# dogeplusplus/torch-actor-critic

Measured on AMD Instinct MI355X. Metric: sac_updates_per_sec, higher is better.
Workload: dtype bf16; 1 GPU; model=SAC-MLP[256, 256]-HalfCheetah-v4, global_batch=64, seq_len=1, parallelism=dp1, obs_dim=17, act_dim=6, replay_buffer=1000000, update_window=50, graph=True, engine=fused, mode=full

## Files before the change

torch_actor_critic_amd/algo/engine.py:

```python

import logging
import math
import os
import typing as t

import torch

from ..buffer.replay import ReplayBuffer
from ..models.mlp import Actor, DoubleCritic
from ..optim import FlatAdam
from ..parallel import comm


_log = logging.getLogger(__name__)


class FusedSACEngine:
    def __init__(self, sac, actor: Actor, critic: DoubleCritic,
                 target_critic: DoubleCritic, buffer: ReplayBuffer,
                 pi_opt: FlatAdam, q_opt: FlatAdam,
                 target_flat: torch.Tensor, batch_size: int,
                 device: torch.device, sample: bool = True,
                 capture: bool = True, philox_seed: int = 0):
        from ..ops import require_extension
# ... 134 lines not shown
                             == "1" and not self._use_side)
        self._wjobs: t.List[tuple] = []
        adam_flag = os.environ.get("TAC_AMD_WGRAD_ADAM", "auto")
        self._wgrad_adam_unsplit = adam_flag == "1"
        self._wgrad_adam = (
            adam_flag != "0"
            and self.world == 1 and not self._force_coll
            and os.environ.get("TAC_AMD_SPLIT_GRAPHS") != "1"
            and self._wgrad_batch)
        self._adam_fused: t.Dict[int, bool] = {}
        self._wt_of = {
            w.grad.data_ptr(): wt
            for w, wt in zip(self._c_tr_src + self._a_tr_src,
                             self._c_tr_dst + self._a_tr_dst)}
        self._bump_fold = os.environ.get("TAC_AMD_BUMP_FOLD", "1") != "0"
        self._r1_dgrad = (
            os.environ.get("TAC_AMD_R1_DGRAD", "1") != "0"
            and len(self.c_w) >= 2 and not self._loss_fuse)
        if self._r1_dgrad and any(self.cwt[z][-1].data_ptr() % 16
                                  for z in range(2)):
            _log.info("engine: rank-1 dgrad operand off (last-layer W^T "
                      "row is not 16-byte aligned); keeping the K=1 launch")
            self._r1_dgrad = False
        self._s2 = torch.cuda.Stream()
        self._fork_evs = [torch.cuda.Event() for _ in range(12)]
        self._join_evs = [torch.cuda.Event() for _ in range(4)]
        self._ev_i = 0
        self._join_i = 0

        torch.cuda.synchronize()

        self._graphs = None
        self.graph = None
        if capture:
            self._capture()


    def _side(self, fn):
        if not self._use_side:
            fn()
            return
        ev = self._fork_evs[self._ev_i % len(self._fork_evs)]
        self._ev_i += 1
        ev.record()
        with torch.cuda.stream(self._s2):
            self._s2.wait_event(ev)
# ... 41 lines not shown
                        [j[6] for j in self._wjobs],
                        [j[7] for j in self._wjobs]) <= 1:
                why = ("the launch does not split along M "
                       "(TAC_AMD_WGRAD_ADAM=1 folds it anyway)")
            if why:
                _log.info("engine: Adam stays in adam_t for the %d-element "
                          "optimizer: %s", g.numel(), why)
            self._adam_fused[key] = why is None
        return self._adam_fused[key]

    def _wflush(self, opt=None, targ=None, rho=0.0):
        if not self._wjobs:
            return
        cols = [list(c) for c in zip(*self._wjobs)]
        if opt is not None and self._adam_covers(opt):
            wts = [self._wt_of.get(dw.data_ptr()) for dw in cols[3]]
            self.ext.mwgrad_het_adam(
                *cols, opt.fp.flat, opt.fp.flat_grad, opt.m, opt.v,
                opt.step_t, opt.lr, opt.betas[0], opt.betas[1], opt.eps,
                opt.weight_decay, wts, targ, rho)
        else:
            self.ext.mwgrad_het(*cols)
        self._wjobs = []

    def _mg(self, xs, ws, bs, ys, masks, M, N, K, lda, ldy, relu,
            xs2=None, ws2=None, masks2=None, K2=0, x_off=0, x2_off=0,
            x_offs=None):
        self.ext.mgemm(xs, ws, bs, ys, masks, M, N, K, lda, ldy, relu,
                       xs2 or [], ws2 or [], masks2 or [], K2, x_off,
                       x2_off, x_offs or [])

    def _critic_fwd(self, x_src, x_off, weights, acts, lda,
                    need_hidden_acts=True):
        B = self.B
        nL = len(self.c_w)
        if self.use_mlpf:
            e = self._empty
            act_arg = [
                [acts[z][i] if (need_hidden_acts or i == nL - 1) else e
                 for i in range(nL)] for z in range(2)]
            self.ext.mlp_fwd_fused(
                x_src, x_off, lda, B, self.OC,
                [[weights[z][i][0] for i in range(nL)] for z in range(2)],
                [[e] * nL for _ in range(2)],
                [[weights[z][i][1] for i in range(nL)] for z in range(2)],
                [[e] * nL for _ in range(2)],
# ... 95 lines not shown
                          self.c_act[0][i], self.c_act[1][i]],
                         [None] * 4, B, self.c_w[i], k, lda, self.c_w[i],
                         relu, x_offs=offs4)
                xs4 = [self.t_act[0][i], self.t_act[1][i],
                       self.c_act[0][i], self.c_act[1][i]]
                offs4 = [0, 0, 0, 0]
                k = self.c_w[i]
                lda = k
        else:
            self._critic_fwd(self.XC, B * self.OCp, self.tw, self.t_act,
                             self.OCp,
                             need_hidden_acts=False)
            self._critic_fwd(self.XC, 0, self.cw, self.c_act, self.OCp)

        nL = len(self.c_w)
        q = [self.c_act[z][nL - 1] for z in range(2)]
        qt = [self.t_act[z][nL - 1] for z in range(2)]
        fuse = self._loss_fuse
        bump = ((self.ctr, self.q_opt.step_t, self.pi_opt.step_t)
                if self._bump_fold else (None, None, None))
        buf = self.buffer
        per = ((self.pprob, buf._size_dev, buf._beta_dev, self.td)
               if self.per else ())
        ext.qloss2(q[0], q[1], qt[0], qt[1], self.logp[B:], self.rew,
                   self.done, self.alpha_dev, self.alpha_host,
                   self.loss_q_acc, self.dq[0], self.dq[1], B,
                   self.sac.gamma, self.sac.reward_scale,
                   self.cwt[0][nL - 1] if fuse else None,
                   self.cwt[1][nL - 1] if fuse else None,
                   self.dc[0][nL - 2] if fuse else None,
                   self.dc[1][nL - 2] if fuse else None,
                   self.c_w[nL - 2] if fuse else 0, *bump, *per)
        if self.per:
            ext.per_update(buf._per_tree, buf.max_size, self.idx, self.td,
                           buf.per_alpha, buf.per_eps, buf._max_priority)

        d = self.dq
        for i in range(nL - 1, -1, -1):
            relu_mask = i + 1 < nL
            masks = [self.c_act[z][i] if relu_mask else None
                     for z in range(2)]
            if i > 0:
                x_in = [self.c_act[z][i - 1] for z in range(2)]
                ldx, xoff = self.c_w[i - 1], 0
            else:
                x_in = [self.XC, self.XC]
                ldx, xoff = self.OCp, 0
            self._wgrad(list(d), list(masks), list(x_in),
                        [self.cw[z][i][0].grad for z in range(2)],
                        [self.cw[z][i][1].grad for z in range(2)],
                        B, self.c_w[i],
                        (self.c_w[i - 1] if i > 0 else OC),
                        self.c_w[i], ldx, xoff)
            if i > 0:
                if i == nL - 1 and fuse:
                    pass
                else:
                    self._mg(d, [self.cwt[z][i] for z in range(2)],
                             [None, None],
                             [self.dc[z][i - 1] for z in range(2)],
                             masks, B, self.c_w[i - 1], self.c_w[i],
                             self.c_w[i], self.c_w[i - 1], False)
                d = [self.dc[z][i - 1] for z in range(2)]
        self._wflush(self.q_opt, self.target_flat, self.sac.polyak)
        self._join_side()

    def _phase_policy(self):
        ext = self.ext
        B, O, A, OC = self.B, self.O, self.A, self.OC
        qo = self.q_opt
        if not self._adam_fused.get(id(qo), False):
            ext.adam_t(qo.fp.flat, qo.fp.flat_grad, qo.m, qo.v, qo.step_t,
                       qo.lr, qo.betas[0], qo.betas[1], qo.eps,
                       qo.weight_decay, self._c_offs, self._c_tr_dst,
                       self.target_flat, self.sac.polyak)

        self._critic_fwd(self.XC2, 0, self.cw, self.p_act, self.OCp)
        nL = len(self.c_w)
        qp = [self.p_act[z][nL - 1] for z in range(2)]
        fuse = self._loss_fuse
        ext.piloss2(qp[0], qp[1], self.logp[:B], self.alpha_dev,
                    self.alpha_host, self.loss_pi_acc, self.mean_logp,
                    self.dqp[0], self.dqp[1], B,
                    self.cwt[0][nL - 1] if fuse else None,
                    self.cwt[1][nL - 1] if fuse else None,
                    self.dcp[0][nL - 2] if fuse else None,
                    self.dcp[1][nL - 2] if fuse else None,
                    self.c_w[nL - 2] if fuse else 0)

        d = self.dqp
        r1 = None
        for i in range(nL - 1, 0, -1):
            masks = [self.p_act[z][i] if i + 1 < nL else None
                     for z in range(2)]
            if i == nL - 1 and fuse:
                d = [self.dcp[z][i - 1] for z in range(2)]
                continue
            if i == nL - 1 and self._r1_dgrad:
                r1 = (list(self.dqp),
                      [self.cwt[z][nL - 1] for z in range(2)])
                continue
            if r1 is not None:
                ext.mgemm_r1(r1[0], r1[1],
                             [self.cwt[z][i] for z in range(2)],
                             [self.dcp[z][i - 1] for z in range(2)], masks,
                             B, self.c_w[i - 1], self.c_w[i],
                             self.c_w[i - 1])
                r1 = None
            else:
                self._mg(d, [self.cwt[z][i] for z in range(2)],
                         [None, None],
                         [self.dcp[z][i - 1] for z in range(2)], masks,
                         B, self.c_w[i - 1], self.c_w[i], self.c_w[i],
                         self.c_w[i - 1], False)
            d = [self.dcp[z][i - 1] for z in range(2)]
        masks0 = [self.p_act[z][0] for z in range(2)]
        if r1 is not None:
            ext.mgemm_r1(r1[0], r1[1], [self.cwt[z][0] for z in range(2)],
                         [self.dxc, self.dxc2], masks0, B, OC, self.c_w[0],
                         self.OCp)
        else:
            self._mg(d, [self.cwt[z][0] for z in range(2)], [None, None],
                     [self.dxc, self.dxc2], masks0,
                     B, OC, self.c_w[0], self.c_w[0], self.OCp, False)

        ext.tg_bwd2(self.dxc, O, self.dxc2, self.alpha_dev,
                    self.alpha_host, self.hl, self.prob, self.dmu,
                    self.dls, B, self.act_limit, self.lo, self.hi)
        h_last = self.a_hidden[-1]
        a_last = self.a_act[-1]
        (wm, bm), (wl, bl) = self.head_w
        self._wgrad([self.dmu, self.dls], [None, None], [a_last, a_last],
                    [wm.grad, wl.grad], [bm.grad, bl.grad],
                    B, A, h_last, A, h_last, 0)
        self._mg([self.dmu], [self.hwt[0]], [None], [self.da[-1]], [None],
                 B, h_last, A, A, h_last, False,
                 xs2=[self.dls], ws2=[self.hwt[1]], masks2=[None], K2=A)

        d = self.da[-1]
        for i in range(len(self.aw) - 1, -1, -1):
            mask = self.a_act[i]
            if i > 0:
                x_in, ldx, xoff = self.a_act[i - 1], self.a_hidden[i - 1], 0
# ... 137 lines not shown
```

torch_actor_critic_amd/ops/csrc/fused.hip:

```cpp

#include <hip/hip_runtime.h>
#include <hip/hip_bf16.h>

#include <torch/extension.h>
#include <c10/hip/HIPStream.h>

#include <algorithm>
#include <utility>
#include <vector>

#include "replay_draw.h"

namespace fused {

using namespace replay;

using f32x4 = __attribute__((ext_vector_type(4))) float;
using bf16x8 = __attribute__((ext_vector_type(8))) __bf16;

__global__ __launch_bounds__(256)
void philox_words2_kernel(int64_t* __restrict__ out, uint64_t seed,
                          uint64_t chi, uint64_t clo0, int64_t n) {
  philox_words_row(out, seed, chi, clo0, n);
}
// ... 451 lines not shown
}

__global__ __launch_bounds__(256)
void mgemm_combine_kernel(MGemm g, int split, bool relu) {
  const int64_t per = (int64_t)g.M * g.N;
  const int64_t total = per * g.nz;
  const int64_t stride = (int64_t)gridDim.x * blockDim.x;
  for (int64_t i = (int64_t)blockIdx.x * blockDim.x + threadIdx.x;
       i < total; i += stride) {
    const int z = (int)(i / per);
    const int64_t off = i % per;
    float s = 0.f;
    for (int sl = 0; sl < split; ++sl)
      s += g.part[((int64_t)sl * g.nz + z) * per + off];
    const MProb& p = g.p[z];
    const int m = (int)(off / g.N), n = (int)(off % g.N);
    if (p.bias) s += p.bias[n];
    if (relu) s = fmaxf(s, 0.f);
    p.y[(int64_t)m * g.ldy + n] = s;
  }
}


constexpr int SKMAX = 256;
constexpr int SLPAD = 8;

DEVINL bool small_vec_ok(const float* src, const float* mask, int r0, int R,
                         int bound, int K, int ld) {
  return (r0 + R <= bound) && ((ld & 3) == 0) && ((K & 3) == 0)
         && ((((uintptr_t)src | (uintptr_t)mask) & 15) == 0);
}

template <int R, bool MASK, bool R1>
DEVINL void small_load(float (&v)[R], float (&mk)[MASK ? R : 1],
                       float (&ra)[R / 16], bool vec,
                       const float* src, const float* mask,
                       int r0, int bound, int K, int ld,
                       const float* r1c, const float* r1r) {
  const int tid = threadIdx.x;
  if (vec) {
    constexpr int G = 64 / R;
    constexpr int NQ = SKMAX / 16 / G;
    const int gr = r0 + ((tid >> 2) & (R - 1));
    const int kg = (tid >> 2) / R;
    const int c = tid & 3;
    if constexpr (R1) ra[0] = r1c[gr];
    const float* base = R1 ? r1r : src + (int64_t)gr * ld;
    const float* mbase = MASK ? mask + (int64_t)gr * ld : nullptr;
#pragma unroll
    for (int q = 0; q < NQ; ++q) {
      if (q * G * 16 < K) {
        const int col = min(((q * G + kg) * 4 + c) * 4, K - 4);
        float4 f = *(const float4*)(base + col);
        v[q*4+0] = f.x; v[q*4+1] = f.y; v[q*4+2] = f.z; v[q*4+3] = f.w;
        if constexpr (MASK) {
          float4 h = *(const float4*)(mbase + col);
          mk[q*4+0] = h.x; mk[q*4+1] = h.y; mk[q*4+2] = h.z; mk[q*4+3] = h.w;
        }
      } else {
#pragma unroll
        for (int j = 0; j < 4; ++j) {
          v[q*4+j] = 0.f;
          if constexpr (MASK) mk[q*4+j] = 0.f;
        }
      }
    }
  } else {
    const int rr = tid >> 4;
    const int cc = tid & 15;
#pragma unroll
    for (int p = 0; p < R / 16; ++p) {
      const bool rows_in = r0 + 16 * p < bound;
      const int gr = min(r0 + rr + 16 * p, bound - 1);
      if constexpr (R1) ra[p] = r1c[gr];
#pragma unroll
      for (int q = 0; q < SKMAX / 16; ++q) {
        if (rows_in && q * 16 < K) {
          const int col = min(cc + 16 * q, K - 1);
          if constexpr (R1) v[p*16+q] = r1r[col];
          else v[p*16+q] = src[(int64_t)gr * ld + col];
          if constexpr (MASK) mk[p*16+q] = mask[(int64_t)gr * ld + col];
        } else {
          v[p*16+q] = 0.f;
          if constexpr (MASK) mk[p*16+q] = 0.f;
        }
      }
    }
  }
}

template <int R, bool MASK, bool R1>
DEVINL void small_write(__bf16* d, int S, const float (&v)[R],
                        const float (&mk)[MASK ? R : 1],
                        const float (&ra)[R / 16], bool vec,
                        int r0, int bound, int K, int Kp) {
  const int tid = threadIdx.x;
  if (vec) {
// ... 19 lines not shown
      }
    }
  } else {
    const int rr = tid >> 4;
    const int cc = tid & 15;
#pragma unroll
    for (int p = 0; p < R / 16; ++p) {
      const int row = rr + 16 * p;
      const bool row_in = r0 + row < bound;
#pragma unroll
      for (int q = 0; q < SKMAX / 16; ++q) {
        if (q * 16 < Kp) {
          const int col = cc + 16 * q;
          float x = v[p*16+q];
          if constexpr (R1) x = ra[p] * x;
          if constexpr (MASK) x = mk[p*16+q] > 0.f ? x : 0.f;
          d[row * S + col] = (__bf16)((row_in && col < K) ? x : 0.f);
        }
      }
    }
  }
}

template <int TM, int TN, bool MASK, bool RELU, bool SUM2, bool R1>
__global__ __launch_bounds__(256)
void mgemm_small_kernel(MGemm g) {
  static_assert((TM == 32 || TM == 64) && (TN == 32 || TN == 64), "tile");
  static_assert(!(SUM2 && R1), "R1 has no second operand");
  constexpr int WM = TM / 2, WN = TN / 2;
  constexpr int MI = WM / 16, NI = WN / 16;
  constexpr int KT = SUM2 ? 2 * SKMAX : SKMAX;
  __shared__ __attribute__((aligned(16))) __bf16 smem[(TM + TN)
                                                      * (KT + SLPAD)];
  const MProb& p = g.p[blockIdx.z];
  const int tid = threadIdx.x;
  const int lane = tid & 63;
  const int wid = tid >> 6;
  const int wrow = (wid >> 1) * WM;
  const int wcol = (wid & 1) * WN;
  const int bm0 = blockIdx.x * TM;
  const int bn0 = blockIdx.y * TN;
  const int crow = (lane >> 4) * 4, ccol = lane & 15;

  const int Kp1 = (g.K + 31) & ~31;
  const int Kp2 = SUM2 ? ((g.K2 + 31) & ~31) : 0;
  const int S = Kp1 + Kp2 + SLPAD;
  __bf16* xs = smem;
  __bf16* ws = smem + TM * S;

  float bv[NI];
#pragma unroll
  for (int ni = 0; ni < NI; ++ni) {
    const int gcol = bn0 + wcol + ni * 16 + ccol;
    bv[ni] = (p.bias && gcol < g.N) ? p.bias[gcol] : 0.f;
  }
  float va[TM], ma[MASK ? TM : 1], ra[TM / 16], vb[TN], nomask[1],
        rb[TN / 16];
  const float* a_src = R1 ? p.r1_row : p.x;
  const bool veca = small_vec_ok(a_src, MASK ? p.mask : nullptr, bm0, TM,
                                 g.M, g.K, g.lda);
  const bool vecb = small_vec_ok(p.w, nullptr, bn0, TN, g.N, g.K, g.K);
  small_load<TM, MASK, R1>(va, ma, ra, veca, p.x, p.mask, bm0, g.M, g.K,
                           g.lda, p.r1_col, p.r1_row);
  small_load<TN, false, false>(vb, nomask, rb, vecb, p.w, nullptr, bn0, g.N,
                               g.K, g.K, nullptr, nullptr);
  float va2[SUM2 ? TM : 1], ma2[(SUM2 && MASK) ? TM : 1], vb2[SUM2 ? TN : 1];
  bool veca2 = false, vecb2 = false;
  if constexpr (SUM2) {
    veca2 = small_vec_ok(p.x2, MASK ? p.mask2 : nullptr, bm0, TM, g.M, g.K2,
                         g.K2);
    vecb2 = small_vec_ok(p.w2, nullptr, bn0, TN, g.N, g.K2, g.K2);
    small_load<TM, MASK, false>(va2, ma2, ra, veca2, p.x2, p.mask2, bm0, g.M,
                                g.K2, g.K2, nullptr, nullptr);
    small_load<TN, false, false>(vb2, nomask, rb, vecb2, p.w2, nullptr, bn0,
                                 g.N, g.K2, g.K2, nullptr, nullptr);
  }

  small_write<TM, MASK, R1>(xs, S, va, ma, ra, veca, bm0, g.M, g.K, Kp1);
  small_write<TN, false, false>(ws, S, vb, nomask, rb, vecb, bn0, g.N, g.K,
                                Kp1);
  if constexpr (SUM2) {
    small_write<TM, MASK, false>(xs + Kp1, S, va2, ma2, ra, veca2, bm0, g.M,
                                 g.K2, Kp2);
    small_write<TN, false, false>(ws + Kp1, S, vb2, nomask, rb, vecb2, bn0,
                                  g.N, g.K2, Kp2);
  }
  __syncthreads();

  f32x4 acc[MI][NI] = {};
  const int arow = lane & 15;
  const int ak0 = (lane >> 4) * 8;
  const __bf16* xr = xs + (wrow + arow) * S + ak0;
  const __bf16* wr = ws + (wcol + arow) * S + ak0;
  const int Kt = Kp1 + Kp2;
  for (int kk = 0; kk < Kt; kk += 32) {
    bf16x8 b[NI];
#pragma unroll
    for (int ni = 0; ni < NI; ++ni)
      b[ni] = *(const bf16x8*)&wr[ni * 16 * S + kk];
#pragma unroll
// ... 825 lines not shown

constexpr int LOSS_MAXB = 1024;

template <bool WEIGHTED>
__global__ __launch_bounds__(256)
void qloss2_kernel(const float* __restrict__ q1, const float* __restrict__ q2,
                   const float* __restrict__ q1t, const float* __restrict__ q2t,
                   const float* __restrict__ logp_next,
                   const float* __restrict__ rew, const float* __restrict__ done,
                   const float* __restrict__ alpha_dev, float alpha_host,
                   float* __restrict__ loss_acc,
                   float* __restrict__ dq1, float* __restrict__ dq2,
                   int B, float gamma, float scale,
                   const float* __restrict__ wt3_0,
                   const float* __restrict__ wt3_1,
                   float* __restrict__ dy2_0, float* __restrict__ dy2_1,
                   int h2,
                   int64_t* __restrict__ bump0, int64_t* __restrict__ bump1,
                   int64_t* __restrict__ bump2,
                   const float* __restrict__ prob,
                   const int64_t* __restrict__ size_dev,
                   const float* __restrict__ beta_dev,
                   float* __restrict__ td) {
  __shared__ float red[4];
  __shared__ float dqs[2][LOSS_MAXB];
  const float alpha = alpha_dev ? alpha_dev[0] : alpha_host;
  const bool fuse = dy2_0 != nullptr;
  int64_t c0 = 0, c1 = 0, c2 = 0;
  if (threadIdx.x == 0) {
    if (bump0) c0 = bump0[0];
    if (bump1) c1 = bump1[0];
    if (bump2) c2 = bump2[0];
  }
  float wsize = 0.f, nbeta = 0.f, wmax = 1.f;
  if constexpr (WEIGHTED) {
    __shared__ float redw[4];
    wsize = (float)size_dev[0];
    nbeta = -beta_dev[0];
    float m = 0.f;
    for (int i = threadIdx.x; i < B; i += blockDim.x)
      m = fmaxf(m, powf(wsize * prob[i], nbeta));
#pragma unroll
    for (int off = 32; off > 0; off >>= 1) m = fmaxf(m, __shfl_down(m, off));
    if ((threadIdx.x & 63) == 0) redw[threadIdx.x >> 6] = m;
    __syncthreads();
    wmax = fmaxf(fmaxf(redw[0], redw[1]), fmaxf(redw[2], redw[3]));
  }
  float acc = 0.f;
  for (int i = threadIdx.x; i < B; i += blockDim.x) {
    float backup = scale * rew[i] + gamma * (1.f - done[i]) *
                       (fminf(q1t[i], q2t[i]) - alpha * logp_next[i]);
    float e1 = q1[i] - backup, e2 = q2[i] - backup;
    float g1, g2;
    if constexpr (WEIGHTED) {
      const float w = powf(wsize * prob[i], nbeta) / wmax;
      acc += w * (e1 * e1 + e2 * e2);
      g1 = 2.f * (w * e1) / B;
      g2 = 2.f * (w * e2) / B;
      td[i] = 0.5f * (fabsf(e1) + fabsf(e2));
    } else {
      acc += e1 * e1 + e2 * e2;
      g1 = 2.f * e1 / B;
      g2 = 2.f * e2 / B;
    }
    dq1[i] = g1;
    dq2[i] = g2;
    if (fuse) { dqs[0][i] = g1; dqs[1][i] = g2; }
  }
#pragma unroll
  for (int off = 32; off > 0; off >>= 1) acc += __shfl_down(acc, off);
  if ((threadIdx.x & 63) == 0) red[threadIdx.x >> 6] = acc;
  __syncthreads();
  if (threadIdx.x == 0) {
    loss_acc[0] += (red[0] + red[1] + red[2] + red[3]) / B;
    if (bump0) bump0[0] = c0 + 1;
    if (bump1) bump1[0] = c1 + 1;
    if (bump2) bump2[0] = c2 + 1;
  }
  if (fuse) {
    const int64_t total = (int64_t)B * h2;
    for (int64_t idx = threadIdx.x; idx < total; idx += blockDim.x) {
      int i = (int)(idx / h2), j = (int)(idx % h2);
      dy2_0[idx] = dqs[0][i] * wt3_0[j];
      dy2_1[idx] = dqs[1][i] * wt3_1[j];
    }
  }
}

__global__ __launch_bounds__(256)
void piloss2_kernel(const float* __restrict__ q1, const float* __restrict__ q2,
                    const float* __restrict__ logp,
                    const float* __restrict__ alpha_dev, float alpha_host,
                    float* __restrict__ loss_acc,
                    float* __restrict__ mean_logp,
                    float* __restrict__ dq1, float* __restrict__ dq2,
                    int B,
                    const float* __restrict__ wt3_0,
                    const float* __restrict__ wt3_1,
                    float* __restrict__ dy2_0, float* __restrict__ dy2_1,
                    int h2) {
  __shared__ float red[4], redl[4];
  __shared__ float dqs[2][LOSS_MAXB];
  const float alpha = alpha_dev ? alpha_dev[0] : alpha_host;
  const bool fuse = dy2_0 != nullptr;
  float acc = 0.f, laux = 0.f;
  for (int i = threadIdx.x; i < B; i += blockDim.x) {
    float a = q1[i], b = q2[i];
    acc += alpha * logp[i] - fminf(a, b);
    laux += logp[i];
    float g1, g2;
    if (a < b)      { g1 = -1.f; g2 = 0.f; }
    else if (b < a) { g1 = 0.f;  g2 = -1.f; }
    else            { g1 = -0.5f; g2 = -0.5f; }
    dq1[i] = g1 / B;
    dq2[i] = g2 / B;
    if (fuse) { dqs[0][i] = g1 / B; dqs[1][i] = g2 / B; }
  }
#pragma unroll
  for (int off = 32; off > 0; off >>= 1) {
    acc += __shfl_down(acc, off);
    laux += __shfl_down(laux, off);
  }
  if ((threadIdx.x & 63) == 0) {
    red[threadIdx.x >> 6] = acc;
    redl[threadIdx.x >> 6] = laux;
  }
  __syncthreads();
  if (threadIdx.x == 0) {
    loss_acc[0] += (red[0] + red[1] + red[2] + red[3]) / B;
    if (mean_logp)
      mean_logp[0] = (redl[0] + redl[1] + redl[2] + redl[3]) / B;
  }
  if (fuse) {
    const int64_t total = (int64_t)B * h2;
    for (int64_t idx = threadIdx.x; idx < total; idx += blockDim.x) {
      int i = (int)(idx / h2), j = (int)(idx % h2);
      dy2_0[idx] = dqs[0][i] * wt3_0[j];
      dy2_1[idx] = dqs[1][i] * wt3_1[j];
    }
  }
}


constexpr int ACT_MAXL = 4;
constexpr int ACT_MAXW = 512;

struct ActArgs {
  const float* x;
  const float* w[ACT_MAXL];
  const float* b[ACT_MAXL];
  int width[ACT_MAXL];
  int n_layers, O, A;
  const float* wmu; const float* bmu;
  const float* wls; const float* bls;
// ... 1039 lines not shown
  const bool fuse = need_fuse(wt3_0, wt3_1, dy2_0, dy2_1, B, h2, "piloss2");
  need_f32(q1, B, "piloss2", "q1");
  need_f32(q2, B, "piloss2", "q2");
  need_f32(logp, B, "piloss2", "logp");
  need_f32(dq1, B, "piloss2", "dq1");
  need_f32(dq2, B, "piloss2", "dq2");
  need_scalar_f32(loss_acc, "piloss2", "loss_acc");
  if (alpha_dev.has_value())
    need_scalar_f32(*alpha_dev, "piloss2", "alpha_dev");
  if (mean_logp.has_value())
    need_scalar_f32(*mean_logp, "piloss2", "mean_logp");
  hipLaunchKernelGGL(piloss2_kernel, dim3(1), dim3(256), 0, stream(),
                     q1.data_ptr<float>(), q2.data_ptr<float>(),
                     logp.data_ptr<float>(), fptr(alpha_dev),
                     (float)alpha_host, loss_acc.data_ptr<float>(),
                     mean_logp.has_value() ? mean_logp->data_ptr<float>()
                                           : nullptr,
                     dq1.data_ptr<float>(), dq2.data_ptr<float>(), (int)B,
                     fptr(wt3_0), fptr(wt3_1),
                     fuse ? dy2_0->data_ptr<float>() : nullptr,
                     fuse ? dy2_1->data_ptr<float>() : nullptr, (int)h2);
}

void adam_t(torch::Tensor p, torch::Tensor g, torch::Tensor m,
            torch::Tensor v, torch::Tensor step, double lr, double b1,
            double b2, double eps, double wd,
            std::vector<int64_t> offsets, std::vector<torch::Tensor> wts,
            c10::optional<torch::Tensor> targ, double rho,
            std::vector<int64_t> bss) {
  ATArgs ta{};
  ta.n_layers = (int)offsets.size();
  TORCH_CHECK(ta.n_layers <= MAX_T);
  TORCH_CHECK(wts.size() == offsets.size(),
              "adam_t: one W^T cache per slab offset");
  TORCH_CHECK(bss.empty() || bss.size() == offsets.size(),
              "adam_t: bss must be empty or hold one entry per slab");
  int64_t slab_end = 0;
  for (int i = 0; i < ta.n_layers; ++i) {
    TORCH_CHECK(offsets[i] >= slab_end,
                "adam_t: slab offsets must be strictly increasing and the "
                "slabs must not overlap (slab ", i, ")");
    slab_end = offsets[i] + wts[i].numel();
    TORCH_CHECK(wts[i].numel() > 0 && slab_end <= p.numel(),
                "adam_t: slab ", i, " does not lie inside [0, n)");
  }
  for (int i = 0; i < ta.n_layers; ++i) {
// ... 241 lines not shown
void alpha_update(torch::Tensor log_alpha, torch::Tensor alpha_dev,
                  torch::Tensor m, torch::Tensor v, torch::Tensor step,
                  torch::Tensor mean_logp, double target_entropy, double lr) {
  need_scalar_f32(log_alpha, "alpha_update", "log_alpha");
  need_scalar_f32(alpha_dev, "alpha_update", "alpha_dev");
  need_scalar_f32(m, "alpha_update", "m");
  need_scalar_f32(v, "alpha_update", "v");
  need_scalar_i64(step, "alpha_update", "step");
  need_scalar_f32(mean_logp, "alpha_update", "mean_logp");
  hipLaunchKernelGGL(alpha_update_kernel, dim3(1), dim3(1), 0, stream(),
                     log_alpha.data_ptr<float>(), alpha_dev.data_ptr<float>(),
                     m.data_ptr<float>(), v.data_ptr<float>(),
                     step.data_ptr<int64_t>(), mean_logp.data_ptr<float>(),
                     (float)target_entropy, (float)lr);
}

}

void register_fused(pybind11::module_& m) {
  m.def("mgemm", &fused::mgemm,
        "multi-problem MFMA GEMM (fwd-form, strided, masked, sum2)");
  m.def("mgemm_r1", &fused::mgemm_r1,
        "masked GEMM whose A operand is a rank-1 product formed on read");
  m.def("mgemm_small_mode", &fused::mgemm_small_mode,
        "set TAC_AMD_MGEMM_SMALL's mode (0 = pipelined kernel only), "
        "returns the previous mode");
  m.def("mwgrad", &fused::mwgrad, "multi-problem wgrad + fused db");
  m.def("mwgrad_het", &fused::mwgrad_het,
        "heterogeneous multi-problem wgrad: one launch per phase");
  m.def("mwgrad_het_adam", &fused::mwgrad_het_adam,
        "heterogeneous wgrad with Adam (+polyak, +W^T) in the epilogue");
  m.def("mwgrad_het_adam_split", &fused::mwgrad_het_adam_split,
        "host-only: M slabs mwgrad_het_adam would use for these shapes");
  m.def("ranges_tile_exactly", &fused::ranges_tile_exactly,
        "host-only: do [off, off+len) ranges tile [0, n) exactly once");
  m.def("transpose_multi", &fused::transpose_multi,
        pybind11::arg("ws"), pybind11::arg("wts"),
        pybind11::arg("blocks") = std::vector<int64_t>{});
  namespace py = pybind11;
  m.def("gather2", &fused::gather2, py::arg("state"), py::arg("act"),
        py::arg("rew"), py::arg("nstate"), py::arg("done"),
        py::arg("size_dev"), py::arg("ctr"), py::arg("seed"), py::arg("xc"),
        py::arg("xc2"), py::arg("orew"), py::arg("od"), py::arg("B"),
        py::arg("ctr_add") = 0);
  m.def("gather2n", &fused::gather2n, py::arg("state"), py::arg("act"),
        py::arg("rew"), py::arg("nstate"), py::arg("done"),
// ... 53 lines not shown
```

Before: 6681 updates/s.

## Fold Q-loss into the critic's rank-1 dgrad GEMM launch

Adds small-GEMM kernel variants that compute the critic Q-loss (and optionally the policy loss) per row and form the rank-1 dgrad operand directly from it. Block 0 also does the loss reduction and the step-counter bumps. This removes the separate qloss2 launch and the K=1 dgrad launch on the critic path, which is on by default. The policy-loss fold stays behind an env flag. In exchange the loss inputs are reloaded per tile, and it relies on M fitting one block and on the small-shape gate.

```diff
diff --git a/torch_actor_critic_amd/algo/engine.py b/torch_actor_critic_amd/algo/engine.py
--- a/torch_actor_critic_amd/algo/engine.py
+++ b/torch_actor_critic_amd/algo/engine.py
@@ -180,6 +180,13 @@
             _log.info("engine: rank-1 dgrad operand off (last-layer W^T "
                       "row is not 16-byte aligned); keeping the K=1 launch")
             self._r1_dgrad = False
+        self._qloss_fold_req = (
+            os.environ.get("TAC_AMD_QLOSS_FOLD", "1") != "0")
+        self._piloss_fold_req = (
+            os.environ.get("TAC_AMD_PILOSS_FOLD", "0") == "1")
+        self._qloss_fold = False
+        self._piloss_fold = False
+        self._fold_ok = self.ext.mgemm_r1_fold_ok
         self._s2 = torch.cuda.Stream()
         self._fork_evs = [torch.cuda.Event() for _ in range(12)]
         self._join_evs = [torch.cuda.Event() for _ in range(4)]
@@ -267,6 +274,25 @@
         else:
             self.ext.mwgrad_het(*cols)
         self._wjobs = []
+
+    def _fold_q(self) -> bool:
+        nL = len(self.c_w)
+        ok = (self._qloss_fold_req and nL >= 3 and not self.per
+              and not self._loss_fuse and self._wgrad_batch
+              and all(self.cwt[z][nL - 1].data_ptr() % 16 == 0
+                      and self.dc[z][nL - 2].data_ptr() % 16 == 0
+                      for z in range(2))
+              and self._fold_ok(self.B, self.c_w[nL - 2]))
+        self._qloss_fold = bool(ok)
+        return self._qloss_fold
+
+    def _fold_pi(self) -> bool:
+        nL = len(self.c_w)
+        ok = (self._piloss_fold_req and self._r1_dgrad
+              and not self._loss_fuse
+              and self._fold_ok(self.B, self.c_w[nL - 2]))
+        self._piloss_fold = bool(ok)
+        return self._piloss_fold
 
     def _mg(self, xs, ws, bs, ys, masks, M, N, K, lda, ldy, relu,
             xs2=None, ws2=None, masks2=None, K2=0, x_off=0, x2_off=0,
@@ -408,15 +434,17 @@
         buf = self.buffer
         per = ((self.pprob, buf._size_dev, buf._beta_dev, self.td)
                if self.per else ())
-        ext.qloss2(q[0], q[1], qt[0], qt[1], self.logp[B:], self.rew,
-                   self.done, self.alpha_dev, self.alpha_host,
-                   self.loss_q_acc, self.dq[0], self.dq[1], B,
-                   self.sac.gamma, self.sac.reward_scale,
-                   self.cwt[0][nL - 1] if fuse else None,
-                   self.cwt[1][nL - 1] if fuse else None,
-                   self.dc[0][nL - 2] if fuse else None,
-                   self.dc[1][nL - 2] if fuse else None,
-                   self.c_w[nL - 2] if fuse else 0, *bump, *per)
+        qfold = self._fold_q()
+        if not qfold:
+            ext.qloss2(q[0], q[1], qt[0], qt[1], self.logp[B:], self.rew,
+                       self.done, self.alpha_dev, self.alpha_host,
+                       self.loss_q_acc, self.dq[0], self.dq[1], B,
+                       self.sac.gamma, self.sac.reward_scale,
+                       self.cwt[0][nL - 1] if fuse else None,
+                       self.cwt[1][nL - 1] if fuse else None,
+                       self.dc[0][nL - 2] if fuse else None,
+                       self.dc[1][nL - 2] if fuse else None,
+                       self.c_w[nL - 2] if fuse else 0, *bump, *per)
         if self.per:
             ext.per_update(buf._per_tree, buf.max_size, self.idx, self.td,
                            buf.per_alpha, buf.per_eps, buf._max_priority)
@@ -439,8 +467,19 @@
                         (self.c_w[i - 1] if i > 0 else OC),
                         self.c_w[i], ldx, xoff)
             if i > 0:
-                if i == nL - 1 and fuse:
+                if i == nL - 1 and (fuse or qfold):
                     pass
+                elif i == nL - 2 and qfold:
+                    ext.mgemm_r1_qloss(
+                        q[0], q[1], qt[0], qt[1], self.logp[B:], self.rew,
+                        self.done, self.alpha_dev, self.alpha_host,
+                        self.loss_q_acc, self.dq[0], self.dq[1],
+                        self.sac.gamma, self.sac.reward_scale, *bump,
+                        [self.cwt[z][nL - 1] for z in range(2)],
+                        [self.cwt[z][i] for z in range(2)],
+                        [self.dc[z][i - 1] for z in range(2)], masks,
+                        [self.dc[z][i] for z in range(2)],
+                        B, self.c_w[i - 1], self.c_w[i], self.c_w[i - 1])
                 else:
                     self._mg(d, [self.cwt[z][i] for z in range(2)],
                              [None, None],
@@ -465,14 +504,25 @@
         nL = len(self.c_w)
         qp = [self.p_act[z][nL - 1] for z in range(2)]
         fuse = self._loss_fuse
-        ext.piloss2(qp[0], qp[1], self.logp[:B], self.alpha_dev,
+        pfold = self._fold_pi()
+        if not pfold:
+            ext.piloss2(qp[0], qp[1], self.logp[:B], self.alpha_dev,
+                        self.alpha_host, self.loss_pi_acc, self.mean_logp,
+                        self.dqp[0], self.dqp[1], B,
+                        self.cwt[0][nL - 1] if fuse else None,
+                        self.cwt[1][nL - 1] if fuse else None,
+                        self.dcp[0][nL - 2] if fuse else None,
+                        self.dcp[1][nL - 2] if fuse else None,
+                        self.c_w[nL - 2] if fuse else 0)
+
+        def r1_gemm(cols, rows, ws, ys, masks, M, N, K, ldy):
+            if pfold:
+                ext.mgemm_r1_piloss(
+                    qp[0], qp[1], self.logp[:B], self.alpha_dev,
                     self.alpha_host, self.loss_pi_acc, self.mean_logp,
-                    self.dqp[0], self.dqp[1], B,
-                    self.cwt[0][nL - 1] if fuse else None,
-                    self.cwt[1][nL - 1] if fuse else None,
-                    self.dcp[0][nL - 2] if fuse else None,
-                    self.dcp[1][nL - 2] if fuse else None,
-                    self.c_w[nL - 2] if fuse else 0)
+                    cols[0], cols[1], rows, ws, ys, masks, M, N, K, ldy)
+            else:
+                ext.mgemm_r1(cols, rows, ws, ys, masks, M, N, K, ldy)
 
         d = self.dqp
         r1 = None
@@ -487,11 +537,10 @@
                       [self.cwt[z][nL - 1] for z in range(2)])
                 continue
             if r1 is not None:
-                ext.mgemm_r1(r1[0], r1[1],
-                             [self.cwt[z][i] for z in range(2)],
-                             [self.dcp[z][i - 1] for z in range(2)], masks,
-                             B, self.c_w[i - 1], self.c_w[i],
-                             self.c_w[i - 1])
+                r1_gemm(r1[0], r1[1],
+                        [self.cwt[z][i] for z in range(2)],
+                        [self.dcp[z][i - 1] for z in range(2)], masks,
+                        B, self.c_w[i - 1], self.c_w[i], self.c_w[i - 1])
                 r1 = None
             else:
                 self._mg(d, [self.cwt[z][i] for z in range(2)],
@@ -502,9 +551,9 @@
             d = [self.dcp[z][i - 1] for z in range(2)]
         masks0 = [self.p_act[z][0] for z in range(2)]
         if r1 is not None:
-            ext.mgemm_r1(r1[0], r1[1], [self.cwt[z][0] for z in range(2)],
-                         [self.dxc, self.dxc2], masks0, B, OC, self.c_w[0],
-                         self.OCp)
+            r1_gemm(r1[0], r1[1], [self.cwt[z][0] for z in range(2)],
+                    [self.dxc, self.dxc2], masks0, B, OC, self.c_w[0],
+                    self.OCp)
         else:
             self._mg(d, [self.cwt[z][0] for z in range(2)], [None, None],
                      [self.dxc, self.dxc2], masks0,
diff --git a/torch_actor_critic_amd/ops/csrc/fused.hip b/torch_actor_critic_amd/ops/csrc/fused.hip
--- a/torch_actor_critic_amd/ops/csrc/fused.hip
+++ b/torch_actor_critic_amd/ops/csrc/fused.hip
@@ -497,6 +497,96 @@
 }
 
 
+struct QRow { float g1, g2, sq; };
+
+DEVINL QRow qloss_row(float q1, float q2, float q1t, float q2t, float lpn,
+                      float rew, float done, float alpha, float gamma,
+                      float scale, int B) {
+#pragma clang fp contract(off)
+  const float soft = __builtin_fmaf(-alpha, lpn, fminf(q1t, q2t));
+  const float backup = scale * rew + gamma * (1.f - done) * soft;
+  const float e1 = q1 - backup, e2 = q2 - backup;
+  QRow r;
+  r.sq = e1 * e1 + e2 * e2;
+  r.g1 = 2.f * e1 / B;
+  r.g2 = 2.f * e2 / B;
+  return r;
+}
+
+struct PiRow { float g1, g2, s; };
+
+DEVINL PiRow piloss_row(float q1, float q2, float lp, float alpha, int B) {
+#pragma clang fp contract(off)
+  PiRow r;
+  r.s = __builtin_fmaf(alpha, lp, -fminf(q1, q2));
+  float g1, g2;
+  if (q1 < q2)      { g1 = -1.f; g2 = 0.f; }
+  else if (q2 < q1) { g1 = 0.f;  g2 = -1.f; }
+  else              { g1 = -0.5f; g2 = -0.5f; }
+  r.g1 = g1 / B;
+  r.g2 = g2 / B;
+  return r;
+}
+
+struct QIn {
+  const float* q1; const float* q2; const float* q1t; const float* q2t;
+  const float* lpn; const float* rew; const float* done;
+};
+
+struct QVals { float q1, q2, q1t, q2t, lpn, rew, done; };
+
+DEVINL QVals qvals_load(const QIn& in, int i) {
+  return QVals{in.q1[i], in.q2[i], in.q1t[i], in.q2t[i], in.lpn[i],
+               in.rew[i], in.done[i]};
+}
+
+template <class L, class F>
+DEVINL float qloss_rows(L&& load, float alpha, float gamma, float scale,
+                        int B, F&& each) {
+#pragma clang fp contract(off)
+  float acc = 0.f;
+  for (int i = threadIdx.x; i < B; i += blockDim.x) {
+    const QVals v = load(i);
+    const QRow r = qloss_row(v.q1, v.q2, v.q1t, v.q2t, v.lpn, v.rew, v.done,
+                             alpha, gamma, scale, B);
+    acc += r.sq;
+    each(i, r);
+  }
+  return acc;
+}
+
+template <class L, class F>
+DEVINL void piloss_rows(float (&acc)[2], L&& load, float alpha, int B,
+                        F&& each) {
+#pragma clang fp contract(off)
+  acc[0] = 0.f;
+  acc[1] = 0.f;
+  for (int i = threadIdx.x; i < B; i += blockDim.x) {
+    const QVals v = load(i);
+    const PiRow r = piloss_row(v.q1, v.q2, v.lpn, alpha, B);
+    acc[0] += r.s;
+    acc[1] += v.lpn;
+    each(i, r);
+  }
+}
+
+template <int N>
+DEVINL void loss_block_mean(float (&acc)[N], float (*red)[4], int B) {
+#pragma clang fp contract(off)
+#pragma unroll
+  for (int off = 32; off > 0; off >>= 1)
+#pragma unroll
+    for (int n = 0; n < N; ++n) acc[n] += __shfl_down(acc[n], off);
+  if ((threadIdx.x & 63) == 0)
+#pragma unroll
+    for (int n = 0; n < N; ++n) red[n][threadIdx.x >> 6] = acc[n];
+  __syncthreads();
+#pragma unroll
+  for (int n = 0; n < N; ++n)
+    acc[n] = (red[n][0] + red[n][1] + red[n][2] + red[n][3]) / B;
+}
+
+
 constexpr int SKMAX = 256;
 constexpr int SLPAD = 8;
 
@@ -506,7 +596,7 @@
          && ((((uintptr_t)src | (uintptr_t)mask) & 15) == 0);
 }
 
-template <int R, bool MASK, bool R1>
+template <int R, bool MASK, bool R1, int LF = 0>
 DEVINL void small_load(float (&v)[R], float (&mk)[MASK ? R : 1],
                        float (&ra)[R / 16], bool vec,
                        const float* src, const float* mask,
@@ -519,7 +609,7 @@
     const int gr = r0 + ((tid >> 2) & (R - 1));
     const int kg = (tid >> 2) / R;
     const int c = tid & 3;
-    if constexpr (R1) ra[0] = r1c[gr];
+    if constexpr (R1 && LF == 0) ra[0] = r1c[gr];
     const float* base = R1 ? r1r : src + (int64_t)gr * ld;
     const float* mbase = MASK ? mask + (int64_t)gr * ld : nullptr;
 #pragma unroll
@@ -547,7 +637,7 @@
     for (int p = 0; p < R / 16; ++p) {
       const bool rows_in = r0 + 16 * p < bound;
       const int gr = min(r0 + rr + 16 * p, bound - 1);
-      if constexpr (R1) ra[p] = r1c[gr];
+      if constexpr (R1 && LF == 0) ra[p] = r1c[gr];
 #pragma unroll
       for (int q = 0; q < SKMAX / 16; ++q) {
         if (rows_in && q * 16 < K) {
@@ -613,11 +703,119 @@
   }
 }
 
-template <int TM, int TN, bool MASK, bool RELU, bool SUM2, bool R1>
+struct LossFold {
+  QIn in;
+  const float* alpha_dev; float alpha_host;
+  float gamma, scale;
+  float* loss_acc;
+  float* mean_logp;
+  float* dq[2];
+  float* outer[2];
+  int64_t* bump[3];
+};
+
+struct FoldPre { QVals v; float loss0; int64_t c[3]; };
+
+template <int LF>
+DEVINL void fold_preload(FoldPre& pre, const LossFold& lf, int B) {
+  const int i = threadIdx.x;
+  if (i < B) {
+    pre.v.q1 = lf.in.q1[i];
+    pre.v.q2 = lf.in.q2[i];
+    pre.v.lpn = lf.in.lpn[i];
+    if constexpr (LF == 2) {
+      pre.v.q1t = lf.in.q1t[i];
+      pre.v.q2t = lf.in.q2t[i];
+      pre.v.rew = lf.in.rew[i];
+      pre.v.done = lf.in.done[i];
+    }
+  }
+  if (i == 0) {
+    pre.loss0 = lf.loss_acc[0];
+    if constexpr (LF == 2) {
+#pragma unroll
+      for (int j = 0; j < 3; ++j)
+        if (lf.bump[j]) pre.c[j] = lf.bump[j][0];
+    }
+  }
+}
+
+template <int LF>
+DEVINL void fold_reduce(const FoldPre& pre, const LossFold& lf, float alpha,
+                        int B) {
+  __shared__ float red[2][4];
+  auto load = [&](int) { return pre.v; };
+  if constexpr (LF == 2) {
+    float acc[1];
+    acc[0] = qloss_rows(load, alpha, lf.gamma, lf.scale, B,
+                        [](int, const QRow&) {});
+    loss_block_mean<1>(acc, red, B);
+    if (threadIdx.x == 0) {
+      lf.loss_acc[0] = pre.loss0 + acc[0];
+#pragma unroll
+      for (int j = 0; j < 3; ++j)
+        if (lf.bump[j]) lf.bump[j][0] = pre.c[j] + 1;
+    }
+  } else {
+    float acc[2];
+    piloss_rows(acc, load, alpha, B, [](int, const PiRow&) {});
+    loss_block_mean<2>(acc, red, B);
+    if (threadIdx.x == 0) {
+      lf.loss_acc[0] = pre.loss0 + acc[0];
+      if (lf.mean_logp) lf.mean_logp[0] = acc[1];
+    }
+  }
+}
+
+template <int R>
+DEVINL void fold_store_outer(float* dst, const float (&v)[R],
+                             const float (&ra)[R / 16], bool vec, int r0,
+                             int bound, int K) {
+  const int tid = threadIdx.x;
+  if (vec) {
+    constexpr int G = 64 / R;
+    constexpr int NQ = SKMAX / 16 / G;
+    const int gr = r0 + ((tid >> 2) & (R - 1));
+    const int kg = (tid >> 2) / R;
+    const int c = tid & 3;
+#pragma unroll
+    for (int q = 0; q < NQ; ++q) {
+      const int col = ((q * G + kg) * 4 + c) * 4;
+      if (q * G * 16 < K && col < K) {
+        float4 f;
+        f.x = ra[0] * v[q*4+0] + 0.f; f.y = ra[0] * v[q*4+1] + 0.f;
+        f.z = ra[0] * v[q*4+2] + 0.f; f.w = ra[0] * v[q*4+3] + 0.f;
+        *(float4*)(dst + (int64_t)gr * K + col) = f;
+      }
+    }
+  } else {
+    const int rr = tid >> 4;
+    const int cc = tid & 15;
+#pragma unroll
+    for (int p = 0; p < R / 16; ++p) {
+      const int gr = r0 + rr + 16 * p;
+#pragma unroll
+      for (int q = 0; q < SKMAX / 16; ++q) {
+        const int col = cc + 16 * q;
+        if (gr < bound && col < K)
+          dst[(int64_t)gr * K + col] = ra[p] * v[p*16+q] + 0.f;
+      }
+    }
+  }
+}
+
+DEVINL float bf16_round(float x) { return (float)(__bf16)x; }
+
+DEVINL const LossFold& fold_arg(const LossFold& lf) { return lf; }
+
+template <int TM, int TN, bool MASK, bool RELU, bool SUM2, bool R1,
+          int LF = 0, class... Fold>
 __global__ __launch_bounds__(256)
-void mgemm_small_kernel(MGemm g) {
+void mgemm_small_kernel(MGemm g, Fold... fold) {
+  static_assert(sizeof...(Fold) == (LF != 0 ? 1 : 0), "one LossFold iff LF");
   static_assert((TM == 32 || TM == 64) && (TN == 32 || TN == 64), "tile");
   static_assert(!(SUM2 && R1), "R1 has no second operand");
+  static_assert(LF == 0 || (R1 && MASK), "a computed column is an R1 column");
   constexpr int WM = TM / 2, WN = TN / 2;
   constexpr int MI = WM / 16, NI = WN / 16;
   constexpr int KT = SUM2 ? 2 * SKMAX : SKMAX;
@@ -651,8 +849,33 @@
   const bool veca = small_vec_ok(a_src, MASK ? p.mask : nullptr, bm0, TM,
                                  g.M, g.K, g.lda);
   const bool vecb = small_vec_ok(p.w, nullptr, bn0, TN, g.N, g.K, g.K);
-  small_load<TM, MASK, R1>(va, ma, ra, veca, p.x, p.mask, bm0, g.M, g.K,
-                           g.lda, p.r1_col, p.r1_row);
+  small_load<TM, MASK, R1, LF>(va, ma, ra, veca, p.x, p.mask, bm0, g.M, g.K,
+                               g.lda, p.r1_col, p.r1_row);
+  constexpr int NFR = LF ? TM / 16 : 1;
+  int frow[NFR];
+  float fin[NFR][LF == 2 ? 7 : 2];
+  float falpha = 0.f;
+  FoldPre fpre = {};
+  if constexpr (LF != 0) {
+    const LossFold& lf = fold_arg(fold...);
+    falpha = lf.alpha_dev ? lf.alpha_dev[0] : lf.alpha_host;
+#pragma unroll
+    for (int q = 0; q < NFR; ++q) {
+      frow[q] = veca ? bm0 + ((tid >> 2) & (TM - 1))
+                     : min(bm0 + (tid >> 4) + 16 * q, g.M - 1);
+      fin[q][0] = lf.in.q1[frow[q]];
+      fin[q][1] = lf.in.q2[frow[q]];
+      if constexpr (LF == 2) {
+        fin[q][2] = lf.in.q1t[frow[q]];
+        fin[q][3] = lf.in.q2t[frow[q]];
+        fin[q][4] = lf.in.lpn[frow[q]];
+        fin[q][5] = lf.in.rew[frow[q]];
+        fin[q][6] = lf.in.done[frow[q]];
+      }
+    }
+    if (blockIdx.x == 0 && blockIdx.y == 0 && blockIdx.z == 0)
+      fold_preload<LF>(fpre, lf, g.M);
+  }
   small_load<TN, false, false>(vb, nomask, rb, vecb, p.w, nullptr, bn0, g.N,
                                g.K, g.K, nullptr, nullptr);
   float va2[SUM2 ? TM : 1], ma2[(SUM2 && MASK) ? TM : 1], vb2[SUM2 ? TN : 1];
@@ -667,6 +890,37 @@
                                  g.N, g.K2, g.K2, nullptr, nullptr);
   }
 
+  if constexpr (LF != 0) {
+    const LossFold& lf = fold_arg(fold...);
+    const int z = blockIdx.z;
+    const bool wr = blockIdx.y == 0
+                    && (veca ? (tid & 3) == 0 && (tid >> 2) / TM == 0
+                             : (tid & 15) == 0);
+#pragma unroll
+    for (int q = 0; q < NFR; ++q) {
+      float col;
+      if constexpr (LF == 2) {
+        const QRow r = qloss_row(fin[q][0], fin[q][1], fin[q][2], fin[q][3],
+                                 fin[q][4], fin[q][5], fin[q][6], falpha,
+                                 lf.gamma, lf.scale, g.M);
+        col = z ? r.g2 : r.g1;
+      } else {
+        const PiRow r = piloss_row(fin[q][0], fin[q][1], 0.f, falpha, g.M);
+        col = z ? r.g2 : r.g1;
+      }
+      const bool row_in = veca ? q == 0 : bm0 + (tid >> 4) + 16 * q < g.M;
+      if (wr && row_in) lf.dq[z][frow[q]] = col;
+      ra[q] = LF == 2 ? bf16_round(col) : col;
+    }
+    if constexpr (LF == 2) {
+#pragma unroll
+      for (int e = 0; e < TM; ++e) va[e] = bf16_round(va[e]);
+      if (blockIdx.y == 0)
+        fold_store_outer<TM>(lf.outer[z], va, ra, veca, bm0, g.M, g.K);
+    }
+    if (blockIdx.x == 0 && blockIdx.y == 0 && blockIdx.z == 0)
+      fold_reduce<LF>(fpre, lf, falpha, g.M);
+  }
   small_write<TM, MASK, R1>(xs, S, va, ma, ra, veca, bm0, g.M, g.K, Kp1);
   small_write<TN, false, false>(ws, S, vb, nomask, rb, vecb, bn0, g.N, g.K,
                                 Kp1);
@@ -1538,7 +1792,7 @@
                    const int64_t* __restrict__ size_dev,
                    const float* __restrict__ beta_dev,
                    float* __restrict__ td) {
-  __shared__ float red[4];
+  __shared__ float red[1][4];
   __shared__ float dqs[2][LOSS_MAXB];
   const float alpha = alpha_dev ? alpha_dev[0] : alpha_host;
   const bool fuse = dy2_0 != nullptr;
@@ -1563,32 +1817,33 @@
     wmax = fmaxf(fmaxf(redw[0], redw[1]), fmaxf(redw[2], redw[3]));
   }
   float acc = 0.f;
-  for (int i = threadIdx.x; i < B; i += blockDim.x) {
-    float backup = scale * rew[i] + gamma * (1.f - done[i]) *
-                       (fminf(q1t[i], q2t[i]) - alpha * logp_next[i]);
-    float e1 = q1[i] - backup, e2 = q2[i] - backup;
-    float g1, g2;
-    if constexpr (WEIGHTED) {
+  if constexpr (WEIGHTED) {
+    for (int i = threadIdx.x; i < B; i += blockDim.x) {
+      float backup = scale * rew[i] + gamma * (1.f - done[i]) *
+                         (fminf(q1t[i], q2t[i]) - alpha * logp_next[i]);
+      float e1 = q1[i] - backup, e2 = q2[i] - backup;
       const float w = powf(wsize * prob[i], nbeta) / wmax;
       acc += w * (e1 * e1 + e2 * e2);
-      g1 = 2.f * (w * e1) / B;
-      g2 = 2.f * (w * e2) / B;
+      const float g1 = 2.f * (w * e1) / B;
+      const float g2 = 2.f * (w * e2) / B;
       td[i] = 0.5f * (fabsf(e1) + fabsf(e2));
-    } else {
-      acc += e1 * e1 + e2 * e2;
-      g1 = 2.f * e1 / B;
-      g2 = 2.f * e2 / B;
-    }
-    dq1[i] = g1;
-    dq2[i] = g2;
-    if (fuse) { dqs[0][i] = g1; dqs[1][i] = g2; }
-  }
-#pragma unroll
-  for (int off = 32; off > 0; off >>= 1) acc += __shfl_down(acc, off);
-  if ((threadIdx.x & 63) == 0) red[threadIdx.x >> 6] = acc;
-  __syncthreads();
+      dq1[i] = g1;
+      dq2[i] = g2;
+      if (fuse) { dqs[0][i] = g1; dqs[1][i] = g2; }
+    }
+  } else {
+    const QIn in{q1, q2, q1t, q2t, logp_next, rew, done};
+    auto load = [&](int i) { return qvals_load(in, i); };
+    acc = qloss_rows(load, alpha, gamma, scale, B, [&](int i, const QRow& r) {
+      dq1[i] = r.g1;
+      dq2[i] = r.g2;
+      if (fuse) { dqs[0][i] = r.g1; dqs[1][i] = r.g2; }
+    });
+  }
+  float mean[1] = {acc};
+  loss_block_mean<1>(mean, red, B);
   if (threadIdx.x == 0) {
-    loss_acc[0] += (red[0] + red[1] + red[2] + red[3]) / B;
+    loss_acc[0] += mean[0];
     if (bump0) bump0[0] = c0 + 1;
     if (bump1) bump1[0] = c1 + 1;
     if (bump2) bump2[0] = c2 + 1;
@@ -1615,37 +1870,25 @@
                     const float* __restrict__ wt3_1,
                     float* __restrict__ dy2_0, float* __restrict__ dy2_1,
                     int h2) {
-  __shared__ float red[4], redl[4];
+  __shared__ float red[2][4];
   __shared__ float dqs[2][LOSS_MAXB];
   const float alpha = alpha_dev ? alpha_dev[0] : alpha_host;
   const bool fuse = dy2_0 != nullptr;
-  float acc = 0.f, laux = 0.f;
-  for (int i = threadIdx.x; i < B; i += blockDim.x) {
-    float a = q1[i], b = q2[i];
-    acc += alpha * logp[i] - fminf(a, b);
-    laux += logp[i];
-    float g1, g2;
-    if (a < b)      { g1 = -1.f; g2 = 0.f; }
-    else if (b < a) { g1 = 0.f;  g2 = -1.f; }
-    else            { g1 = -0.5f; g2 = -0.5f; }
-    dq1[i] = g1 / B;
-    dq2[i] = g2 / B;
-    if (fuse) { dqs[0][i] = g1 / B; dqs[1][i] = g2 / B; }
-  }
-#pragma unroll
-  for (int off = 32; off > 0; off >>= 1) {
-    acc += __shfl_down(acc, off);
-    laux += __shfl_down(laux, off);
-  }
-  if ((threadIdx.x & 63) == 0) {
-    red[threadIdx.x >> 6] = acc;
-    redl[threadIdx.x >> 6] = laux;
-  }
-  __syncthreads();
+  float acc[2];
+  auto load = [&](int i) {
+    QVals v = {};
+    v.q1 = q1[i]; v.q2 = q2[i]; v.lpn = logp[i];
+    return v;
+  };
+  piloss_rows(acc, load, alpha, B, [&](int i, const PiRow& r) {
+    dq1[i] = r.g1;
+    dq2[i] = r.g2;
+    if (fuse) { dqs[0][i] = r.g1; dqs[1][i] = r.g2; }
+  });
+  loss_block_mean<2>(acc, red, B);
   if (threadIdx.x == 0) {
-    loss_acc[0] += (red[0] + red[1] + red[2] + red[3]) / B;
-    if (mean_logp)
-      mean_logp[0] = (redl[0] + redl[1] + redl[2] + redl[3]) / B;
+    loss_acc[0] += acc[0];
+    if (mean_logp) mean_logp[0] = acc[1];
   }
   if (fuse) {
     const int64_t total = (int64_t)B * h2;
@@ -2731,6 +2974,156 @@
                      fuse ? dy2_1->data_ptr<float>() : nullptr, (int)h2);
 }
 
+
+bool mgemm_r1_fold_ok(int64_t M, int64_t K) {
+  return M >= 1 && K >= 1 && small_gate(*g_bf16_flag, 1, 1, M, K, false, 0);
+}
+
+static void fold_gemm_args(MGemm& g, const char* op,
+                           const std::vector<torch::Tensor>& rows,
+                           const std::vector<torch::Tensor>& ws,
+                           const std::vector<torch::Tensor>& ys,
+                           const std::vector<torch::Tensor>& masks,
+                           int64_t M, int64_t N, int64_t K, int64_t ldy) {
+  TORCH_CHECK(rows.size() == 2 && ws.size() == 2 && ys.size() == 2
+              && masks.size() == 2, op, ": exactly 2 problems (nz == 2)");
+  TORCH_CHECK(M >= 1 && N >= 1 && K >= 1 && ldy >= N, op, ": shape");
+  TORCH_CHECK(mgemm_r1_fold_ok(M, K), op, ": outside the small-shape gate "
+              "(bf16 compute, M <= 128, K <= ", SKMAX, ", small mode on)");
+  g.M = (int)M; g.N = (int)N; g.K = (int)K;
+  g.lda = (int)K; g.ldy = (int)ldy;
+  g.nz = 2; g.k_chunk = (int)K; g.part = nullptr;
+  for (int z = 0; z < 2; ++z) {
+    need_f32(rows[z], 0, op, "row");
+    TORCH_CHECK(rows[z].numel() == K
+                && ((uintptr_t)rows[z].data_ptr<float>() & 15) == 0,
+                op, ": row ", z, " must be K floats, 16-byte aligned");
+    need_f32(ws[z], 0, op, "w");
+    TORCH_CHECK(ws[z].numel() == N * K, op, ": w ", z);
+    need_f32(masks[z], 0, op, "mask");
+    TORCH_CHECK(masks[z].numel() == M * K, op, ": mask ", z);
+    TORCH_CHECK(ys[z].is_cuda() && ys[z].scalar_type() == torch::kFloat32
+                && ys[z].numel() >= (M - 1) * ldy + N, op, ": y ", z);
+    g.p[z].r1_row = rows[z].data_ptr<float>();
+    g.p[z].w = ws[z].data_ptr<float>();
+    g.p[z].y = ys[z].data_ptr<float>();
+    g.p[z].mask = masks[z].data_ptr<float>();
+  }
+}
+
+static void need_vecM(const torch::Tensor& t, int64_t M, const char* op,
+                      const char* name) {
+  need_f32(t, M, op, name);
+  TORCH_CHECK(t.numel() == M, op, ": ", name, " must hold M = ", M,
+              " elements");
+}
+
+template <int LF>
+static void launch_small_fold(const MGemm& g, const LossFold& lf) {
+  constexpr int T = 32;
+  TORCH_CHECK(g.M <= 256, "folded loss: M must not exceed the block size");
+  dim3 grid((unsigned)((g.M + T - 1) / T), (unsigned)((g.N + T - 1) / T), 2);
+  hipLaunchKernelGGL((mgemm_small_kernel<T, T, true, false, false, true, LF,
+                                         LossFold>),
+                     grid, dim3(256), 0, stream(), g, lf);
+}
+
+void mgemm_r1_qloss(torch::Tensor q1, torch::Tensor q2, torch::Tensor q1t,
+                    torch::Tensor q2t, torch::Tensor logp_next,
+                    torch::Tensor rew, torch::Tensor done,
+                    c10::optional<torch::Tensor> alpha_dev, double alpha_host,
+                    torch::Tensor loss_acc, torch::Tensor dq1,
+                    torch::Tensor dq2, double gamma, double scale,
+                    c10::optional<torch::Tensor> bump0,
+                    c10::optional<torch::Tensor> bump1,
+                    c10::optional<torch::Tensor> bump2,
+                    std::vector<torch::Tensor> rows,
+                    std::vector<torch::Tensor> ws,
+                    std::vector<torch::Tensor> ys,
+                    std::vector<torch::Tensor> masks,
+                    std::vector<torch::Tensor> outers,
+                    int64_t M, int64_t N, int64_t K, int64_t ldy) {
+  const char* op = "mgemm_r1_qloss";
+  MGemm g{};
+  fold_gemm_args(g, op, rows, ws, ys, masks, M, N, K, ldy);
+  need_vecM(q1, M, op, "q1");
+  need_vecM(q2, M, op, "q2");
+  need_vecM(q1t, M, op, "q1t");
+  need_vecM(q2t, M, op, "q2t");
+  need_vecM(logp_next, M, op, "logp_next");
+  need_vecM(rew, M, op, "rew");
+  need_vecM(done, M, op, "done");
+  need_vecM(dq1, M, op, "dq1");
+  need_vecM(dq2, M, op, "dq2");
+  need_scalar_f32(loss_acc, op, "loss_acc");
+  if (alpha_dev.has_value()) need_scalar_f32(*alpha_dev, op, "alpha_dev");
+  if (bump0.has_value()) need_scalar_i64(*bump0, op, "bump0");
+  if (bump1.has_value()) need_scalar_i64(*bump1, op, "bump1");
+  if (bump2.has_value()) need_scalar_i64(*bump2, op, "bump2");
+  TORCH_CHECK(outers.size() == 2, op, ": exactly 2 outer-product buffers");
+  for (int z = 0; z < 2; ++z) {
+    need_f32(outers[z], M * K, op, "outer");
+    TORCH_CHECK(((uintptr_t)outers[z].data_ptr<float>() & 15) == 0, op,
+                ": outer ", z, " must be 16-byte aligned");
+  }
+  auto iptr = [](const c10::optional<torch::Tensor>& t) -> int64_t* {
+    return t.has_value() ? t->data_ptr<int64_t>() : nullptr;
+  };
+  LossFold lf{};
+  lf.in = QIn{q1.data_ptr<float>(), q2.data_ptr<float>(),
+              q1t.data_ptr<float>(), q2t.data_ptr<float>(),
+              logp_next.data_ptr<float>(), rew.data_ptr<float>(),
+              done.data_ptr<float>()};
+  lf.alpha_dev = fptr(alpha_dev);
+  lf.alpha_host = (float)alpha_host;
+  lf.gamma = (float)gamma;
+  lf.scale = (float)scale;
+  lf.loss_acc = loss_acc.data_ptr<float>();
+  lf.dq[0] = dq1.data_ptr<float>();
+  lf.dq[1] = dq2.data_ptr<float>();
+  lf.outer[0] = outers[0].data_ptr<float>();
+  lf.outer[1] = outers[1].data_ptr<float>();
+  lf.bump[0] = iptr(bump0);
+  lf.bump[1] = iptr(bump1);
+  lf.bump[2] = iptr(bump2);
+  launch_small_fold<2>(g, lf);
+}
+
+void mgemm_r1_piloss(torch::Tensor q1, torch::Tensor q2, torch::Tensor logp,
+                     c10::optional<torch::Tensor> alpha_dev,
+                     double alpha_host, torch::Tensor loss_acc,
+                     c10::optional<torch::Tensor> mean_logp,
+                     torch::Tensor dq1, torch::Tensor dq2,
+                     std::vector<torch::Tensor> rows,
+                     std::vector<torch::Tensor> ws,
+                     std::vector<torch::Tensor> ys,
+                     std::vector<torch::Tensor> masks,
+                     int64_t M, int64_t N, int64_t K, int64_t ldy) {
+  const char* op = "mgemm_r1_piloss";
+  MGemm g{};
+  fold_gemm_args(g, op, rows, ws, ys, masks, M, N, K, ldy);
+  need_vecM(q1, M, op, "q1");
+  need_vecM(q2, M, op, "q2");
+  need_vecM(logp, M, op, "logp");
+  need_vecM(dq1, M, op, "dq1");
+  need_vecM(dq2, M, op, "dq2");
+  need_scalar_f32(loss_acc, op, "loss_acc");
+  if (alpha_dev.has_value()) need_scalar_f32(*alpha_dev, op, "alpha_dev");
+  if (mean_logp.has_value()) need_scalar_f32(*mean_logp, op, "mean_logp");
+  LossFold lf{};
+  lf.in.q1 = q1.data_ptr<float>();
+  lf.in.q2 = q2.data_ptr<float>();
+  lf.in.lpn = logp.data_ptr<float>();
+  lf.alpha_dev = fptr(alpha_dev);
+  lf.alpha_host = (float)alpha_host;
+  lf.loss_acc = loss_acc.data_ptr<float>();
+  lf.mean_logp = mean_logp.has_value() ? mean_logp->data_ptr<float>()
+                                         : nullptr;
+  lf.dq[0] = dq1.data_ptr<float>();
+  lf.dq[1] = dq2.data_ptr<float>();
+  launch_small_fold<1>(g, lf);
+}
+
 void adam_t(torch::Tensor p, torch::Tensor g, torch::Tensor m,
             torch::Tensor v, torch::Tensor step, double lr, double b1,
             double b2, double eps, double wd,
@@ -3018,6 +3411,12 @@
         "multi-problem MFMA GEMM (fwd-form, strided, masked, sum2)");
   m.def("mgemm_r1", &fused::mgemm_r1,
         "masked GEMM whose A operand is a rank-1 product formed on read");
+  m.def("mgemm_r1_qloss", &fused::mgemm_r1_qloss,
+        "qloss2 + K=1 dgrad + masked dgrad in one small-shape launch");
+  m.def("mgemm_r1_piloss", &fused::mgemm_r1_piloss,
+        "piloss2 + mgemm_r1 in one small-shape launch");
+  m.def("mgemm_r1_fold_ok", &fused::mgemm_r1_fold_ok,
+        "host-only: do (M, K) pass the gate of the two folded entries");
   m.def("mgemm_small_mode", &fused::mgemm_small_mode,
         "set TAC_AMD_MGEMM_SMALL's mode (0 = pipelined kernel only), "
         "returns the previous mode");
```

After: 6876 updates/s, median of 6. 2.9% higher.
